# maelaubert/VulkanSift

Hardware: AMD Instinct MI355X
Metric: SIFT detect+match frames/sec (640x480, ~2k kp) (higher is better)
Workload: dtype f32

## Files before the change

include/vksift_hip.h:

```cpp
#ifndef VKSIFT_HIP_H
#define VKSIFT_HIP_H

#include <stddef.h>
#include <stdint.h>

#ifdef __cplusplus
extern "C"
{
#endif

#define VKSIFT_HIP_MAX_TAPS 20
#define VKSIFT_HIP_MATCH_CHUNKS 32
#define VKSIFT_HIP_MATCH_SMALL_NA 1536u
#define VKSIFT_HIP_MATCH_SMALL_NB 4096u
#define VKSIFT_HIP_MATCH_SCRATCH_U32(na, nb) (2u * (size_t)(na) + (size_t)(nb) + 72u + (size_t)(na) * 16u * VKSIFT_HIP_MATCH_CHUNKS)
#define VKSIFT_HIP_ABI_VERSION 6u
#define VKSIFT_HIP_GATHER_SLOTS 512u
#define VKSIFT_HIP_MATCH_SLOTS 256u
#define VKSIFT_HIP_MATCH_PK_NB 32768u
#define VKSIFT_HIP_MAX_ORI 18
#define VKSIFT_HIP_MAX_OCTAVE_SIDE 16383u

  typedef void *vksift_hip_stream;
  typedef void *vksift_hip_graph;
  typedef void *vksift_hip_event;

  int vksift_hip_init(void);
  uint32_t vksift_hip_abi_version(void);
  int vksift_hip_device_count(void);
  int vksift_hip_device_name(int idx, char *out256);
  int vksift_hip_set_device(int idx);
  size_t vksift_hip_device_free_mem(void);
  void *vksift_hip_malloc(size_t bytes);
  void vksift_hip_free(void *p);
  void *vksift_hip_host_malloc(size_t bytes);
  void vksift_hip_host_free(void *p);
  int vksift_hip_host_register(void *p, size_t bytes);
  int vksift_hip_host_unregister(void *p);
  int vksift_hip_is_pinned(const void *p);
  vksift_hip_stream vksift_hip_stream_create(void);
  void vksift_hip_stream_destroy(vksift_hip_stream s);
  int vksift_hip_stream_sync(vksift_hip_stream s);
  int vksift_hip_stream_busy(vksift_hip_stream s);
  vksift_hip_event vksift_hip_event_create(void);
  void vksift_hip_event_destroy(vksift_hip_event e);
  int vksift_hip_event_record(vksift_hip_event e, vksift_hip_stream s);
  int vksift_hip_event_sync(vksift_hip_event e);
  int vksift_hip_event_busy(vksift_hip_event e);
  float vksift_hip_event_elapsed_ms(vksift_hip_event a, vksift_hip_event b);
  int vksift_hip_stream_wait_event(vksift_hip_stream s, vksift_hip_event e);
  int vksift_hip_capture_begin(vksift_hip_stream s);
  int vksift_hip_capture_end(vksift_hip_stream s, vksift_hip_graph *out);
  int vksift_hip_graph_launch(vksift_hip_graph g, vksift_hip_stream s);
  void vksift_hip_graph_destroy(vksift_hip_graph g);
  int vksift_hip_memcpy_h2d(void *dst, const void *src, size_t n, vksift_hip_stream s);
  int vksift_hip_memcpy_d2h(void *dst, const void *src, size_t n, vksift_hip_stream s);
  int vksift_hip_memcpy_d2d(void *dst, const void *src, size_t n, vksift_hip_stream s);
  int vksift_hip_memcpy2d_d2h(void *dst, size_t dpitch, const void *src, size_t spitch, size_t width_bytes, size_t height, vksift_hip_stream s);
  int vksift_hip_post_words(uint32_t *host_mapped_dst, const uint32_t *src, size_t n_words, vksift_hip_stream s);
  int vksift_hip_memset(void *dst, int value, size_t n, vksift_hip_stream s);
  const char *vksift_hip_error_string(int err);
  void vksift_hip_range_push(const char *name);
  void vksift_hip_range_pop(void);

  enum
  {
    VKSIFT_TUNE_WG_TARGET = 0,
    VKSIFT_TUNE_WIDE_MASK = 1,
    VKSIFT_TUNE_MULTI_MAX = 2,
    VKSIFT_TUNE_REFINE_PTR = 3,
    VKSIFT_TUNE_SCAN_FORM = 4,
    VKSIFT_TUNE_PAIR_FORM = 5,
    VKSIFT_TUNE_PYR_GATE = 6,
    VKSIFT_TUNE_DENSE_ROWS = 7,
    VKSIFT_TUNE_SEED_WG = 8,
    VKSIFT_TUNE_SCAN_BAND = 9,
    VKSIFT_TUNE_TAIL_MULTI = 10,
    VKSIFT_TUNE_ZERO_COPY = 11,
    VKSIFT_TUNE_MIN_MARCH = 12,
    VKSIFT_TUNE_COUNT = 16
  };
  int vksift_hip_tune(int knob, int value);
  int vksift_hip_tune_get(int knob);


  typedef struct
  {
    float *base;
    uint32_t w, h;
    uint32_t pitch;
    uint64_t img_stride;
    uint32_t fp16;
    uint32_t reverse;
  } vksift_hip_Plane;

  int vksift_hip_input_blit(const uint8_t *src, uint32_t sw, uint32_t sh, uint64_t src_img_stride, vksift_hip_Plane dst, uint32_t batch,
                            vksift_hip_stream s);

  int vksift_hip_blur(vksift_hip_Plane src, vksift_hip_Plane dst, const float *taps, uint32_t ntaps, uint32_t batch, vksift_hip_stream s);

  int vksift_hip_blur_pair(vksift_hip_Plane src, vksift_hip_Plane dst1, vksift_hip_Plane dst2, const float *taps1, uint32_t ntaps1, const float *taps2,
                           uint32_t ntaps2, uint32_t batch, vksift_hip_stream s);

  int vksift_hip_blur_form(vksift_hip_Plane src, vksift_hip_Plane dst, uint32_t ntaps, uint32_t batch);

  int vksift_hip_blur_multi(const vksift_hip_Plane *src, const vksift_hip_Plane *dst, uint32_t n, const float *taps, uint32_t ntaps, uint32_t batch,
                            vksift_hip_stream s);

  int vksift_hip_blur_downsample(vksift_hip_Plane src, vksift_hip_Plane dst, vksift_hip_Plane next, const float *taps, uint32_t ntaps, uint32_t batch,
                                 vksift_hip_stream s);

  int vksift_hip_seed_upsampled(const uint8_t *src, uint32_t sw, uint32_t sh, uint64_t src_img_stride, vksift_hip_Plane dst, const float *taps, uint32_t ntaps,
                                uint32_t batch, vksift_hip_stream s);

  int vksift_hip_seed_direct(const uint8_t *src, uint32_t sw, uint32_t sh, uint64_t src_img_stride, vksift_hip_Plane dst, const float *taps, uint32_t ntaps,
                             uint32_t batch, vksift_hip_stream s);

  int vksift_hip_downsample(vksift_hip_Plane src, vksift_hip_Plane dst, uint32_t batch, vksift_hip_stream s);

  int vksift_hip_octave_chain(const vksift_hip_Plane *layers, uint32_t n_oct, uint32_t n_layers, uint32_t S, const float *taps, const uint32_t *ntaps,
                              uint32_t batch, vksift_hip_stream s);

  int vksift_hip_dog_plane(const float *lo, const float *hi, uint32_t w, uint32_t h, uint32_t pitch, uint32_t fp16, float *out_dense, vksift_hip_stream s);

  typedef struct
  {
    float *gauss;
    uint32_t fp16;
    uint32_t w, h, pitch;
    uint64_t plane_stride;
    uint64_t img_stride;
    uint32_t S;
    int32_t octave_idx;
    float seed_sigma;
    float dog_threshold;
    float edge_limit;
    uint8_t *feats;
    uint64_t feat_img_stride;
    uint32_t cap;
    uint32_t *found;
    uint32_t found_img_stride;
    uint64_t *seg_mask;
    uint32_t *seg_off;
    uint64_t seg_img_stride;
    uint32_t *cand_xy;
    uint32_t *cand_flag;
    uint32_t *cand_n;
    uint64_t cand_img_stride;
    uint32_t cand_cap;
    float *ori_ang;
    uint32_t *ori_cnt;
    uint64_t ori_img_stride;
    uint32_t max_ori;
    uint32_t use_vlfeat;
    const float *desc_fp_tab;
    uint32_t desc_fp_tab_len;
    uint32_t scan_reverse;
    uint32_t masks_cleared;
    uint32_t sec_index;
  } vksift_hip_OctaveJob;

  typedef struct
  {
    uint8_t *desc;
    uint64_t desc_img_stride;
    uint32_t *norm;
    uint64_t norm_img_stride;
    uint32_t *n;
    uint32_t n_img_stride;
    uint32_t nsec;
    uint32_t sec_cap[16];
    uint8_t *post;
    uint64_t post_img_stride;
    uint32_t *found_post;
    uint32_t found_post_n;
  } vksift_hip_DenseRows;

  int vksift_hip_extract_keypoints(const vksift_hip_OctaveJob *job, uint32_t batch, vksift_hip_stream s, vksift_hip_event scan_done);
  int vksift_hip_orientations(const vksift_hip_OctaveJob *job, uint32_t batch, vksift_hip_stream s);
  int vksift_hip_descriptors(const vksift_hip_OctaveJob *job, uint32_t batch, vksift_hip_stream s);
  int vksift_hip_extract_keypoints_multi(const vksift_hip_OctaveJob *jobs, uint32_t n_jobs, uint32_t batch, vksift_hip_stream s, vksift_hip_event scan_done);
  int vksift_hip_clear_segment_masks(const vksift_hip_OctaveJob *jobs, uint32_t n_jobs, uint32_t batch, vksift_hip_stream s);
  int vksift_hip_selftest_inrange(uint32_t n, uint32_t seed, uint32_t *d_mismatches, vksift_hip_stream s);
  int vksift_hip_orientations_multi(const vksift_hip_OctaveJob *jobs, uint32_t n_jobs, uint32_t batch, vksift_hip_stream s);
  int vksift_hip_descriptors_multi(const vksift_hip_OctaveJob *jobs, uint32_t n_jobs, uint32_t batch, vksift_hip_stream s);
  int vksift_hip_descriptors_multi_dense(const vksift_hip_OctaveJob *jobs, uint32_t n_jobs, uint32_t batch, const vksift_hip_DenseRows *dense,
                                         vksift_hip_stream s);

  int vksift_hip_gather_descriptors(const uint8_t *feats, uint32_t n, uint8_t *desc, vksift_hip_stream s);
  size_t vksift_hip_match_scratch_u32(uint32_t na, uint32_t nb);
  int vksift_hip_match_2nn_desc(const uint8_t *desc_a, uint32_t na, uint32_t a_index_base, const uint8_t *desc_b, uint32_t nb, uint32_t *norm_scratch,
                                size_t scratch_u32, uint8_t *matches, vksift_hip_stream s);
  int vksift_hip_shifted_norms(const uint8_t *desc, uint32_t n, uint32_t *norms, vksift_hip_stream s);
  int vksift_hip_match_2nn_prenormed(const uint8_t *desc_a, const uint32_t *norm_a, uint32_t na, uint32_t a_index_base, const uint8_t *desc_b,
                                     const uint32_t *norm_b, uint32_t nb, uint32_t *scratch, size_t scratch_u32, uint8_t *matches, vksift_hip_stream s);

  int vksift_hip_filter_matches(const uint8_t *fwd, uint64_t fwd_slot_stride, const uint8_t *rev, uint64_t rev_slot_stride, const uint32_t *n_fwd,
                                uint32_t n_stride, float ratio, uint32_t nslots, uint8_t *out, uint64_t out_slot_stride, uint32_t *out_n, vksift_hip_stream s);

  int vksift_hip_pack_features(const uint8_t *feats_base, uint64_t buf_stride, const uint32_t *buf_ids, const uint32_t *out_rows, uint32_t nslots, uint32_t nsec,
                               const uint32_t *sec_off, const uint32_t *sec_cap, const uint32_t *found_base, uint32_t found_buf_stride, uint8_t *out,
                               uint32_t max_rows, uint32_t *found_post, vksift_hip_stream s);
  int vksift_hip_gather_sections(const uint8_t *feats_base, uint64_t buf_stride, const uint32_t *buf_ids, uint32_t nslots, uint32_t nsec,
                                 const uint32_t *sec_off, const uint32_t *sec_cap, const uint32_t *fixed_counts, const uint32_t *found_base,
                                 uint32_t found_buf_stride, uint32_t max_rows, uint32_t pad_rows_to, uint8_t *desc, uint64_t desc_stride,
                                 uint32_t *norms, uint64_t norm_stride, uint32_t *n_out_dev, uint32_t n_stride, vksift_hip_stream s);
  int vksift_hip_match_2nn_async(const uint8_t *cache_desc, const uint32_t *cache_norm, const uint32_t *cache_n, const uint32_t *ids_a, const uint32_t *ids_b,
                                 uint32_t max_na, uint32_t max_nb, uint32_t nb_exact, uint32_t *redo, uint32_t *n_dev, uint8_t *matches, uint32_t nslots, uint64_t cache_desc_stride,
                                 uint64_t cache_norm_stride, uint64_t redo_slot_stride, uint64_t match_slot_stride, uint32_t n_slot_stride,
                                 uint32_t *partial_scratch, vksift_hip_stream s);

  int vksift_hip_gather_correspondences(const uint8_t *feats_base, uint64_t buf_stride, const uint32_t *found_base, uint32_t found_buf_stride,
                                        const uint32_t *slot_tab, const uint32_t *layouts, const uint8_t *filtered, uint64_t filtered_slot_stride,
                                        const uint32_t *filtered_n, uint32_t max_n, uint32_t nslots, float *corr, uint64_t corr_slot_stride, vksift_hip_stream s);
  size_t vksift_hip_ransac_scratch_u32(uint32_t nslots, uint32_t nb_hypotheses);
  int vksift_hip_ransac_homography(const float *corr, uint64_t corr_slot_stride, const uint32_t *n_dev, uint32_t n_stride, uint32_t max_n, uint32_t nslots,
                                   uint32_t nb_hypotheses, float threshold_px, uint64_t seed, uint8_t *results, uint8_t *masks, uint64_t mask_slot_stride,
                                   uint32_t *scratch, size_t scratch_u32, vksift_hip_stream s);
  int vksift_hip_ransac_fundamental(const float *corr, uint64_t corr_slot_stride, const uint32_t *n_dev, uint32_t n_stride, uint32_t max_n, uint32_t nslots,
                                    uint32_t nb_hypotheses, float threshold_px, uint64_t seed, uint8_t *results, uint8_t *masks, uint64_t mask_slot_stride,
                                    uint32_t *scratch, size_t scratch_u32, vksift_hip_stream s);

#define VKSIFT_HIP_GUIDE_HOMOGRAPHY 0u
#define VKSIFT_HIP_GUIDE_FUNDAMENTAL 1u
  int vksift_hip_gather_xy(const uint8_t *feats_base, uint64_t buf_stride, const uint32_t *found_base, uint32_t found_buf_stride, const uint32_t *slot_tab,
                           const uint32_t *layouts, uint32_t max_n, uint32_t nslots, float *xy, uint64_t xy_side_stride, vksift_hip_stream s);
  size_t vksift_hip_guided_scratch_u32(uint32_t nslots, uint32_t max_n);
  int vksift_hip_match_guided(const uint8_t *cache_desc, uint64_t cache_desc_stride, const uint32_t *cache_norm, uint64_t cache_norm_stride, const uint32_t *slot_tab,
                              uint32_t slot_tab_stride, const float *xy, uint64_t xy_side_stride, const uint32_t *n_dev, uint32_t n_stride, uint32_t max_n,
                              const float *models, uint32_t model_stride, const uint32_t *valid, uint32_t valid_stride, uint32_t model_kind, float t2, float ratio,
                              float max_distance, uint32_t cross_check, uint32_t nslots, uint8_t *out, uint64_t out_slot_stride, uint32_t *out_n, uint32_t *scratch,
                              size_t scratch_u32, vksift_hip_stream s);

#ifdef __cplusplus
}
#endif
#endif
```

vulkansift_amd/csrc/hip/extrema.hip:

```cpp
#include <hip/hip_runtime.h>
#include <type_traits>
#include <stdint.h>
#include <stdlib.h>

#include "../detmath.h"
#include "multi.h"
#include "vksift_hip.h"

namespace
{

struct DogView
{
  const float *base;
  int w, h, pitch;
  size_t plane;
  int S;
  int fp16;
};

template <bool F16>
__device__ __forceinline__ float ld(const DogView &d, int s, int x, int y)
{
  if (s < 0 || s > d.S + 1)
// ... 150 lines not shown
    float i33 = ((h11 * h22) - (h12 * h12)) / det;
    oS = -i11 * gS - i12 * gX - i13 * gY;
    oX = -i12 * gS - i22 * gX - i23 * gY;
    oY = -i13 * gS - i23 * gX - i33 * gY;

    if (fabsf(oX) < 0.6f && fabsf(oY) < 0.6f && fabsf(oS) < 0.6f)
      break;
    else if (step < 4)
    {
      rx += ((oX >= 0.6f && rx < (W - 2)) ? 1 : 0) + ((oX <= -0.6f && rx > 1) ? -1 : 0);
      ry += ((oY >= 0.6f && ry < (H - 2)) ? 1 : 0) + ((oY <= -0.6f && ry > 1) ? -1 : 0);
      rs += ((oS >= 0.6f && rs < (S + 1)) ? 1 : 0) + ((oS <= -0.6f && rs > 1) ? -1 : 0);
    }
  }
  float sx = (float)rx + oX, sy = (float)ry + oY, ss = (float)rs + oS;
  float nv = vc + 0.5f * (gX * oX + gY * oY + gS * oS);
  if (!(fabsf(nv) > dog_threshold && fabsf(oX) < 1.5f && fabsf(oY) < 1.5f && fabsf(oS) < 1.5f && sx >= 0 && sx < (float)W && sy >= 0 && sy < (float)H &&
        ss >= 0 && ss <= (float)(S + 1)))
    return false;
  float e11 = xp + xm - 2.f * vc;
  float e22 = yp + ym - 2.f * vc;
  float e12 = h23;
  float edgeness = ((e11 + e22) * (e11 + e22)) / ((e11 * e22) - (e12 * e12));
  if (!((edgeness < edge_limit) && (edgeness >= 0)))
    return false;

  float scale_factor = octave_idx >= 0 ? dm_pow2i(octave_idx) : 1.f / dm_pow2i(-octave_idx);
  kp->scale_x = sx;
  kp->scale_y = sy;
  kp->scale_idx = (uint32_t)roundf(ss);
  kp->octave_idx = octave_idx;
  kp->sigma = seed_sigma * dm_exp2f(ss / (float)S) * scale_factor;
  kp->orientation = 0.f;
  kp->intensity = nv;
  kp->x = sx * scale_factor;
  kp->y = sy * scale_factor;
  return true;
}

struct ExtremaArgs
{
  const float *gauss;
  int fp16;
  int w, h, pitch;
  uint64_t plane_stride, img_stride;
  int S, octave_idx;
  float seed_sigma, dog_threshold, edge_limit;
  uint64_t *seg_mask;
  uint32_t *seg_off;
  uint64_t seg_img_stride;
  int nseg;
  uint8_t *feats;
  uint64_t feat_img_stride;
  uint32_t cap;
  uint32_t *found;
  uint32_t found_img_stride;
  uint32_t *cand_xy;
  uint32_t *cand_flag;
  uint32_t *cand_n;
  uint64_t cand_img_stride;
  uint32_t cand_cap;
  int band;
  uint32_t nsegs;
  uint32_t nchunks;
  int scan_rev;
};

__device__ __forceinline__ float wave_shr1(float v, float edge)
{
  return __builtin_bit_cast(float, __builtin_amdgcn_update_dpp(__builtin_bit_cast(int, edge), __builtin_bit_cast(int, v), 0x138, 0xf, 0xf, false));
}
__device__ __forceinline__ float wave_shl1(float v, float edge)
{
  return __builtin_bit_cast(float, __builtin_amdgcn_update_dpp(__builtin_bit_cast(int, edge), __builtin_bit_cast(int, v), 0x130, 0xf, 0xf, false));
}

__device__ __forceinline__ float fmax2(float a, float b)
{
  float r;
  asm("v_max_f32 %0, %1, %2" : "=v"(r) : "v"(a), "v"(b));
  return r;
}
__device__ __forceinline__ float fmin2(float a, float b)
{
  float r;
  asm("v_min_f32 %0, %1, %2" : "=v"(r) : "v"(a), "v"(b));
  return r;
}
__device__ __forceinline__ float fmax3(float a, float b, float c)
{
  float r;
  asm("v_max3_f32 %0, %1, %2, %3" : "=v"(r) : "v"(a), "v"(b), "v"(c));
  return r;
}
__device__ __forceinline__ float fmin3(float a, float b, float c)
{
  float r;
  asm("v_min3_f32 %0, %1, %2, %3" : "=v"(r) : "v"(a), "v"(b), "v"(c));
  return r;
}

__device__ __forceinline__ unsigned long long spread32(unsigned long long x)
{
  x &= 0xFFFFFFFFull;
  x = (x | (x << 16)) & 0x0000FFFF0000FFFFull;
  x = (x | (x << 8)) & 0x00FF00FF00FF00FFull;
  x = (x | (x << 4)) & 0x0F0F0F0F0F0F0F0Full;
  x = (x | (x << 2)) & 0x3333333333333333ull;
  x = (x | (x << 1)) & 0x5555555555555555ull;
  return x;
}

typedef unsigned u32x2_t __attribute__((ext_vector_type(2)));
constexpr unsigned EXT_OOB = 0x80000000u;

template <int S, int NSLOT, bool F16>
__global__ void __launch_bounds__(256, 4) k_extrema_lean(Multi<ExtremaArgs> m, int strip_major)
{
  const VBlock vb = vblock(m);
  const ExtremaArgs &a = m.oct[vb.o];
  const int band = a.band;
  constexpr int NL = S + 2;
  constexpr int EB = F16 ? 2 : 4;
  constexpr int AHEAD = NSLOT - 3;
  const int lane = threadIdx.x & 63;
  const int wv = __builtin_amdgcn_readfirstlane((int)(threadIdx.x >> 6));
  int b = vb.z;
  int bx = vb.x, by = vb.y * 4 + wv;
  if (strip_major)
  {
    unsigned blk = vb.y * vb.gx + vb.x;
    if (strip_major & 2)
    {
      const unsigned per_img = vb.gx * vb.gy, total = per_img * vb.gz;
      if ((total & 7u) == 0)
      {
        const unsigned n = blk + per_img * vb.z, per = total >> 3, k = n >> 3;
        const unsigned wi = (n & 7u) * per + (a.scan_rev ? per - 1u - k : k);
        b = (int)(wi / per_img);
        blk = wi - (unsigned)b * per_img;
      }
    }
    const unsigned id = blk * 4u + (unsigned)wv, ns = (unsigned)(a.nseg + 1) / 2u;
    by = (int)(id / ns), bx = (int)(id - (unsigned)by * ns);
  }
  const int y0 = by * band;
  if (y0 >= a.h)
    return;
  const int y1 = min(y0 + band, a.h);
  const int x0 = bx * 128, x = x0 + 2 * lane;
  const uint8_t *img = (const uint8_t *)a.gauss + (size_t)b * a.img_stride * EB;
  const int pitch4 = a.pitch * EB;
  __amdgpu_buffer_rsrc_t rs[NL + 1];
#pragma unroll
  for (int l = 0; l <= NL; l++)
    rs[l] = __builtin_amdgcn_make_buffer_rsrc((void *)(img + (size_t)l * a.plane_stride * EB), 0, a.pitch * a.h * EB, 0x00020000);
  const unsigned off2 = x < a.pitch ? (unsigned)x * (unsigned)EB : EXT_OOB;
  const int hx = lane == 0 ? x0 - 1 : x0 + 128;
  const unsigned offh = ((lane == 0 || lane == 63) && hx >= 0 && hx < a.pitch) ? (unsigned)hx * (unsigned)EB : EXT_OOB;
  const unsigned long long colA = __ballot(x >= 1 && x < a.w - 1), colB = __ballot(x + 1 < a.w - 1);
  const float pre = a.dog_threshold * 0.8f;
  const int seg0 = bx * 2;
  const bool has_seg1 = seg0 + 1 < a.nseg;
  const int ylo = max(y0, 1), yhi = min(y1, a.h - 1);
  const bool odd = lane & 1;
  const unsigned half = (unsigned)lane >> 1;

  u32x2_t wv2[NSLOT][NL + 1];
  unsigned wh[NSLOT][NL + 1];
  auto fetch_row = [&](int r, auto SLOT) {
    constexpr int slot = decltype(SLOT)::value;
    const int rr = min(max(r, 0), a.h - 1);
    const int so = rr * pitch4;
#pragma unroll
    for (int l = 0; l <= NL; l++)
    {
      if (F16)
      {
        wv2[slot][l].x = __builtin_amdgcn_raw_buffer_load_b32(rs[l], off2, so, 0);
        wh[slot][l] = (unsigned)__builtin_amdgcn_raw_buffer_load_b16(rs[l], offh, so, 0);
      }
      else
      {
        wv2[slot][l] = __builtin_amdgcn_raw_buffer_load_b64(rs[l], off2, so, 0);
        wh[slot][l] = __builtin_amdgcn_raw_buffer_load_b32(rs[l], offh, so, 0);
      }
    }
  };
  typedef _Float16 h2x __attribute__((ext_vector_type(2)));
  auto to_dog = [&](auto SLOT) {
    constexpr int slot = decltype(SLOT)::value;
    if (F16)
    {
      float lo0, lo1, loh;
      {
        const h2x t = __builtin_bit_cast(h2x, wv2[slot][0].x);
        lo0 = (float)t.x, lo1 = (float)t.y;
        loh = (float)__builtin_bit_cast(h2x, wh[slot][0]).x;
      }
#pragma unroll
      for (int l = 0; l < NL; l++)
      {
        const h2x t = __builtin_bit_cast(h2x, wv2[slot][l + 1].x);
        const float hi0 = (float)t.x, hi1 = (float)t.y, hih = (float)__builtin_bit_cast(h2x, wh[slot][l + 1]).x;
        wv2[slot][l].x = __float_as_uint((float)(_Float16)(hi0 - lo0));
        wv2[slot][l].y = __float_as_uint((float)(_Float16)(hi1 - lo1));
        wh[slot][l] = __float_as_uint((float)(_Float16)(hih - loh));
        lo0 = hi0, lo1 = hi1, loh = hih;
      }
      return;
    }
#pragma unroll
    for (int l = 0; l < NL; l++)
    {
      wv2[slot][l].x = __float_as_uint(__uint_as_float(wv2[slot][l + 1].x) - __uint_as_float(wv2[slot][l].x));
      wv2[slot][l].y = __float_as_uint(__uint_as_float(wv2[slot][l + 1].y) - __uint_as_float(wv2[slot][l].y));
      wh[slot][l] = __float_as_uint(__uint_as_float(wh[slot][l + 1]) - __uint_as_float(wh[slot][l]));
    }
  };

  auto phase = [&](auto PC, int r) {
    constexpr int P = decltype(PC)::value;
    constexpr int sn = P, sm = (P + NSLOT - 1) % NSLOT, so_ = (P + NSLOT - 2) % NSLOT, sf = (P + AHEAD) % NSLOT;
    if (r + AHEAD <= y1)
      fetch_row(r + AHEAD, std::integral_constant<int, sf>{});
    to_dog(std::integral_constant<int, sn>{});
    const int y = r - 1;
    if (y < ylo || y >= yhi)
      return;
    float ownxA[S], ownnA[S], ownxB[S], ownnB[S], fullxA[NL], fullnA[NL], fullxB[NL], fullnB[NL];
#pragma unroll
    for (int l = 0; l < NL; l++)
    {
      const float ao = __uint_as_float(wv2[so_][l].x), am = __uint_as_float(wv2[sm][l].x), an = __uint_as_float(wv2[sn][l].x);
      const float bo = __uint_as_float(wv2[so_][l].y), bm = __uint_as_float(wv2[sm][l].y), bn = __uint_as_float(wv2[sn][l].y);
      const float ho = __uint_as_float(wh[so_][l]), hm = __uint_as_float(wh[sm][l]), hn = __uint_as_float(wh[sn][l]);
      const float vxa = fmax3(ao, am, an), vna = fmin3(ao, am, an);
      const float vxb = fmax3(bo, bm, bn), vnb = fmin3(bo, bm, bn);
      const float vxh = fmax3(ho, hm, hn), vnh = fmin3(ho, hm, hn);
      const float Lx = wave_shr1(vxb, vxh), Ln = wave_shr1(vnb, vnh);
      const float Rx = wave_shl1(vxa, vxh), Rn = wave_shl1(vna, vnh);
      if (l >= 1 && l <= S)
      {
        ownxA[l - 1] = fmax3(Lx, vxb, fmax2(ao, an)), ownnA[l - 1] = fmin3(Ln, vnb, fmin2(ao, an));
        ownxB[l - 1] = fmax3(vxa, Rx, fmax2(bo, bn)), ownnB[l - 1] = fmin3(vna, Rn, fmin2(bo, bn));
      }
      fullxA[l] = fmax3(Lx, vxa, vxb), fullnA[l] = fmin3(Ln, vna, vnb);
      fullxB[l] = fmax3(vxa, vxb, Rx), fullnB[l] = fmin3(vna, vnb, Rn);
    }
#pragma unroll
    for (int sz = 0; sz < S; sz++)
    {
      const int l = sz + 1;
      const float ca = __uint_as_float(wv2[sm][l].x), cb = __uint_as_float(wv2[sm][l].y);
      const float nxa = fmax3(ownxA[sz], fullxA[l - 1], fullxA[l + 1]), nna = fmin3(ownnA[sz], fullnA[l - 1], fullnA[l + 1]);
      const float nxb = fmax3(ownxB[sz], fullxB[l - 1], fullxB[l + 1]), nnb = fmin3(ownnB[sz], fullnB[l - 1], fullnB[l + 1]);
      const unsigned long long ma = (__ballot(ca > nxa) | __ballot(ca < nna)) & __ballot(fabsf(ca) > pre) & colA;
      const unsigned long long mb = (__ballot(cb > nxb) | __ballot(cb < nnb)) & __ballot(fabsf(cb) > pre) & colB;
      if ((ma | mb) != 0ull)
      {
        const unsigned lo = odd ? (unsigned)mb : (unsigned)ma, hi = odd ? (unsigned)(mb >> 32) : (unsigned)(ma >> 32);
        const unsigned long long m0 = __ballot((lo >> half) & 1u), m1 = __ballot((hi >> half) & 1u);
        if (lane == 0)
        {
          const size_t base = ((size_t)sz * a.h + y) * a.nseg + (size_t)b * a.seg_img_stride;
          a.seg_mask[base + seg0] = m0;
          if (has_seg1)
            a.seg_mask[base + seg0 + 1] = m1;
        }
      }
    }
  };

  if (AHEAD >= 1)
    fetch_row(y0 - 1, std::integral_constant<int, 0>{});
  if (AHEAD >= 2)
    fetch_row(y0, std::integral_constant<int, 1 % NSLOT>{});
  int r = y0 - 1;
  for (;;)
  {
    phase(std::integral_constant<int, 0>{}, r);
    if (++r > y1)
      break;
    phase(std::integral_constant<int, 1>{}, r);
    if (++r > y1)
      break;
    phase(std::integral_constant<int, 2>{}, r);
    if (++r > y1)
      break;
    phase(std::integral_constant<int, 3>{}, r);
    if (++r > y1)
      break;
    if (NSLOT > 4)
    {
      phase(std::integral_constant<int, 4 % NSLOT>{}, r);
      if (++r > y1)
        break;
    }
  }
}

constexpr uint32_t SEG_CHUNK = 4096;

__global__ void __launch_bounds__(1024) k_segment_scan(Multi<ExtremaArgs> m)
{
  __shared__ uint32_t wave_tot[16];
  const VBlock vb = vblock(m);
  const ExtremaArgs &a = m.oct[vb.o];
  const int b = (int)vb.y;
  const uint64_t *__restrict__ mask = a.seg_mask + (size_t)b * a.seg_img_stride;
  uint32_t *__restrict__ off = a.seg_off + (size_t)b * a.seg_img_stride;
  uint32_t *__restrict__ chunk_tot = a.cand_flag;
  const uint64_t chunk_img_stride = a.cand_img_stride;
  const uint32_t n = a.nsegs;
  const int lane = threadIdx.x & 63, wave = threadIdx.x >> 6;
  const uint32_t i0 = vb.x * SEG_CHUNK + 4u * threadIdx.x;
  uint32_t p[4];
#pragma unroll
  for (int k = 0; k < 4; k++)
    p[k] = i0 + k < n ? (uint32_t)__popcll(mask[i0 + k]) : 0u;
  const uint32_t tsum = p[0] + p[1] + p[2] + p[3];
  uint32_t incl = tsum;
#pragma unroll
  for (int dlt = 1; dlt < 64; dlt <<= 1)
  {
    uint32_t t = __shfl_up(incl, dlt, 64);
    if (lane >= dlt)
      incl += t;
  }
  if (lane == 63)
    wave_tot[wave] = incl;
  __syncthreads();
  uint32_t wave_base = 0, total = 0;
  for (int wv = 0; wv < 16; wv++)
  {
    if (wv < wave)
      wave_base += wave_tot[wv];
    total += wave_tot[wv];
  }
  uint32_t run = wave_base + incl - tsum;
#pragma unroll
  for (int k = 0; k < 4; k++)
  {
    if (i0 + k < n)
      off[i0 + k] = run;
    run += p[k];
  }
  if (threadIdx.x == 0)
    chunk_tot[(size_t)b * chunk_img_stride + vb.x] = total;
}


__global__ void __launch_bounds__(256) k_cand_list(Multi<ExtremaArgs> mu)
{
  const VBlock vb = vblock(mu);
  const ExtremaArgs &a = mu.oct[vb.o];
  const uint32_t seg = vb.x * 256 + threadIdx.x;
  const int b = (int)vb.y;
  const uint32_t *chunk_tot = a.cand_flag + (size_t)b * a.cand_img_stride;
  if (vb.x == 0 && threadIdx.x == 0)
  {
    uint32_t total = 0;
    for (uint32_t c = 0; c < a.nchunks; c++)
      total += chunk_tot[c];
    a.cand_n[b] = total;
    if (total == 0)
      a.found[(size_t)b * a.found_img_stride] = 0;
  }
  unsigned long long m = seg < a.nsegs ? a.seg_mask[seg + (size_t)b * a.seg_img_stride] : 0ull;
  if (__ballot(m != 0ull) == 0ull)
    return;
  uint32_t base = 0;
  for (uint32_t c = threadIdx.x & 63u, nc = (vb.x * 256u) / SEG_CHUNK; c < nc; c += 64u)
    base += chunk_tot[c];
#pragma unroll
  for (int dlt = 32; dlt >= 1; dlt >>= 1)
    base += __shfl_xor(base, dlt, 64);
  if (m == 0ull)
    return;
  uint32_t pos = a.seg_off[seg + (size_t)b * a.seg_img_stride] + base;
  const uint32_t segx = seg % (uint32_t)a.nseg;
  const uint32_t yy = (seg / (uint32_t)a.nseg) % (uint32_t)a.h;
  const uint32_t sz = seg / ((uint32_t)a.nseg * (uint32_t)a.h);
  uint32_t *out = a.cand_xy + (size_t)b * a.cand_img_stride;
  while (m)
  {
    const int bit = __ffsll((long long)m) - 1;
    m &= m - 1;
    if (pos < a.cand_cap)
      out[pos] = (segx * 64u + (uint32_t)bit) | (yy << 14) | ((sz + 1u) << 28);
    pos++;
  }
}

template <bool F16, bool BUF>
__global__ void __launch_bounds__(256) k_refine_flags(Multi<ExtremaArgs> m)
{
  __shared__ uint32_t s_cnt[4];
  const VBlock vb = vblock(m);
  const ExtremaArgs &a = m.oct[vb.o];
  const int b = (int)vb.x;
  uint32_t n = a.cand_n[b];
  n = n < a.cand_cap ? n : a.cand_cap;
  const uint32_t nch = (n + 255u) / 256u;
  DogView d{(const float *)((const uint8_t *)a.gauss + (size_t)b * a.img_stride * (a.fp16 ? 2u : 4u)), a.w, a.h, a.pitch, (size_t)a.plane_stride, a.S, a.fp16};
  const __amdgpu_buffer_rsrc_t rsrc =
      __builtin_amdgcn_make_buffer_rsrc((void *)d.base, 0, (int)((unsigned)(a.S + 3) * (unsigned)a.plane_stride * (F16 ? 2u : 4u)), 0x00020000);
  const uint32_t *xy = a.cand_xy + (size_t)b * a.cand_img_stride;
  uint32_t *flag = a.cand_flag + (size_t)b * a.cand_img_stride;
  uint32_t *chunk_sum = a.seg_off + (size_t)b * a.seg_img_stride;
  for (uint32_t chunk = vb.y; chunk < nch; chunk += vb.gy)
  {
    const uint32_t i = chunk * 256u + threadIdx.x;
    bool ok = false;
    if (i < n)
    {
      const uint32_t c = xy[i];
      KpRecord kp;
      const int cx = (int)(c & 0x3fffu), cy = (int)((c >> 14) & 0x3fffu), cs = (int)(c >> 28);
      ok = BUF ? refine_texel_buf<F16>(rsrc, a.w, a.h, a.pitch, (unsigned)a.plane_stride, a.S, cx, cy, cs, a.dog_threshold, a.edge_limit, a.seed_sigma, a.octave_idx, &kp)
               : refine_texel<F16>(d, cx, cy, cs, a.dog_threshold, a.edge_limit, a.seed_sigma, a.octave_idx, &kp);
      flag[i] = ok ? 1u : 0u;
    }
    const unsigned long long bal = __ballot(ok);
    if ((threadIdx.x & 63) == 0)
      s_cnt[threadIdx.x >> 6] = (uint32_t)__popcll(bal);
    __syncthreads();
    if (threadIdx.x == 0)
      chunk_sum[chunk] = s_cnt[0] + s_cnt[1] + s_cnt[2] + s_cnt[3];
    __syncthreads();
  }
}

template <bool F16, bool BUF>
__global__ void __launch_bounds__(256) k_cand_emit(Multi<ExtremaArgs> m)
{
  __shared__ uint32_t s_cnt[4];
  __shared__ uint32_t s_red[4];
  __shared__ uint32_t s_list[256];
  const VBlock vb = vblock(m);
  const ExtremaArgs &a = m.oct[vb.o];
  const int b = (int)vb.x;
  const int lane = threadIdx.x & 63, wave = threadIdx.x >> 6;
  uint32_t n = a.cand_n[b];
  n = n < a.cand_cap ? n : a.cand_cap;
  const uint32_t nch = (n + 255u) / 256u;
  DogView d{(const float *)((const uint8_t *)a.gauss + (size_t)b * a.img_stride * (a.fp16 ? 2u : 4u)), a.w, a.h, a.pitch, (size_t)a.plane_stride, a.S, a.fp16};
  const __amdgpu_buffer_rsrc_t rsrc =
      __builtin_amdgcn_make_buffer_rsrc((void *)d.base, 0, (int)((unsigned)(a.S + 3) * (unsigned)a.plane_stride * (F16 ? 2u : 4u)), 0x00020000);
  const uint32_t *xy = a.cand_xy + (size_t)b * a.cand_img_stride;
  const uint32_t *flag = a.cand_flag + (size_t)b * a.cand_img_stride;
  const uint32_t *chunk_sum = a.seg_off + (size_t)b * a.seg_img_stride;
  for (uint32_t chunk = vb.y; chunk < nch; chunk += vb.gy)
  {
    uint32_t part = 0;
    for (uint32_t c = threadIdx.x; c < chunk; c += 256u)
      part += chunk_sum[c];
#pragma unroll
    for (int dlt = 32; dlt >= 1; dlt >>= 1)
      part += __shfl_xor(part, dlt, 64);
    const uint32_t i = chunk * 256u + threadIdx.x;
    const bool v = i < n && flag[i] != 0u;
    const unsigned long long bal = __ballot(v);
    if (lane == 0)
      s_cnt[wave] = (uint32_t)__popcll(bal), s_red[wave] = part;
    __syncthreads();
    const uint32_t cbase = s_red[0] + s_red[1] + s_red[2] + s_red[3];
    uint32_t rank = (uint32_t)__popcll(bal & ((1ull << lane) - 1ull));
    for (int wv = 0; wv < wave; wv++)
      rank += s_cnt[wv];
    const uint32_t total = s_cnt[0] + s_cnt[1] + s_cnt[2] + s_cnt[3];
    if (v)
      s_list[rank] = xy[i];
    __syncthreads();
    const uint32_t idx = cbase + threadIdx.x;
    if (chunk + 1u == nch && threadIdx.x == 0)
      a.found[(size_t)b * a.found_img_stride] = cbase + total;
    if (threadIdx.x < total && idx < a.cap)
    {
      const uint32_t c = s_list[threadIdx.x];
      KpRecord kp;
      const int cx = (int)(c & 0x3fffu), cy = (int)((c >> 14) & 0x3fffu), cs = (int)(c >> 28);
      if (BUF)
        refine_texel_buf<F16>(rsrc, a.w, a.h, a.pitch, (unsigned)a.plane_stride, a.S, cx, cy, cs, a.dog_threshold, a.edge_limit, a.seed_sigma, a.octave_idx, &kp);
      else
        refine_texel<F16>(d, cx, cy, cs, a.dog_threshold, a.edge_limit, a.seed_sigma, a.octave_idx, &kp);
      uint32_t *rec = (uint32_t *)(a.feats + (size_t)b * a.feat_img_stride + (size_t)idx * 164);
      rec[0] = __float_as_uint(kp.x);
      rec[1] = __float_as_uint(kp.y);
      rec[2] = __float_as_uint(kp.scale_x);
      rec[3] = __float_as_uint(kp.scale_y);
      rec[4] = kp.scale_idx;
      rec[5] = (uint32_t)kp.octave_idx;
      rec[6] = __float_as_uint(kp.sigma);
      rec[7] = __float_as_uint(kp.orientation);
      rec[8] = __float_as_uint(kp.intensity);
    }
    __syncthreads();
  }
}

}

static int make_extrema_args(const vksift_hip_OctaveJob *job, ExtremaArgs *out)
{
  if (job->w > VKSIFT_HIP_MAX_OCTAVE_SIDE || job->h > VKSIFT_HIP_MAX_OCTAVE_SIDE || job->S > 14u)
    return (int)hipErrorInvalidValue;
  ExtremaArgs a;
  a.gauss = job->gauss;
  a.fp16 = (int)job->fp16;
  a.w = (int)job->w, a.h = (int)job->h, a.pitch = (int)job->pitch;
  a.plane_stride = job->plane_stride, a.img_stride = job->img_stride;
  a.S = (int)job->S, a.octave_idx = job->octave_idx;
  a.seed_sigma = job->seed_sigma, a.dog_threshold = job->dog_threshold, a.edge_limit = job->edge_limit;
  a.seg_mask = job->seg_mask, a.seg_off = job->seg_off, a.seg_img_stride = job->seg_img_stride;
  a.nseg = (int)((job->w + 63) / 64);
  a.feats = job->feats, a.feat_img_stride = job->feat_img_stride, a.cap = job->cap;
  a.found = job->found, a.found_img_stride = job->found_img_stride;
  a.cand_xy = job->cand_xy, a.cand_flag = job->cand_flag, a.cand_n = job->cand_n;
  a.cand_img_stride = job->cand_img_stride, a.cand_cap = job->cand_cap;
  a.scan_rev = (int)job->scan_reverse;
  a.band = job->h > 256u ? 48 : 16;
  if (vksift_hip_tune_get(VKSIFT_TUNE_SCAN_BAND) > 0 && job->h > 256u)
    a.band = vksift_hip_tune_get(VKSIFT_TUNE_SCAN_BAND);
  a.nsegs = job->S * job->h * (uint32_t)a.nseg;
  a.nchunks = (a.nsegs + SEG_CHUNK - 1u) / SEG_CHUNK;
  if (job->seg_img_stride != a.nsegs || a.nchunks > a.cand_cap)
    return (int)hipErrorInvalidValue;
  *out = a;
  return 0;
}

static int clear_masks(const ExtremaArgs *args, uint32_t n, uint32_t batch, hipStream_t hs)
{
  for (uint32_t i = 0; i < n;)
  {
    uint32_t j = i + 1;
    size_t bytes = sizeof(uint64_t) * (size_t)args[i].nsegs * batch;
    while (j < n && (const uint8_t *)args[j].seg_mask == (const uint8_t *)args[i].seg_mask + bytes)
      bytes += sizeof(uint64_t) * (size_t)args[j].nsegs * batch, j++;
    const hipError_t me = hipMemsetAsync(args[i].seg_mask, 0, bytes, hs);
    if (me != hipSuccess)
      return (int)me;
    i = j;
  }
  return 0;
}

static int extract_run(const vksift_hip_OctaveJob *jobs, uint32_t n, uint32_t batch, hipStream_t hs, hipEvent_t scan_done)
{
  ExtremaArgs args[MULTI_MAX];
  for (uint32_t i = 0; i < n; i++)
  {
    const int e = make_extrema_args(&jobs[i], &args[i]);
    if (e)
      return e;
  }
  const bool f16 = args[0].fp16 != 0;
  const int S = args[0].S;
  {
    uint64_t waves = 0;
    for (uint32_t i = 0; i < n; i++)
      waves += (uint64_t)batch * ((args[i].w + 127) / 128) * ((args[i].h + args[i].band - 1) / args[i].band);
    if (waves < 2048u && vksift_hip_tune_get(VKSIFT_TUNE_SCAN_BAND) <= 0)
      for (uint32_t i = 0; i < n; i++)
        args[i].band = 16;
  }

  bool cleared = true;
  for (uint32_t i = 0; i < n; i++)
    cleared = cleared && jobs[i].masks_cleared != 0;
  if (!cleared)
  {
    const int me = clear_masks(args, n, batch, hs);
    if (me)
      return me;
  }
  const int sm = 3;
  for (uint32_t i = 0; i < n; i++)
    if ((uint64_t)jobs[i].pitch * jobs[i].h * (f16 ? 2u : 4u) >= 0x80000000ull)
      return (int)hipErrorInvalidValue;

#define VKSIFT_MULTI(M, GX, GY, GZ)                              \
  Multi<ExtremaArgs> M;                                           \
  M.n = 0;                                                        \
  for (uint32_t i = 0; i < n; i++)                                \
  {                                                               \
    const ExtremaArgs &a = args[i];                               \
    (void)a;                                                      \
    if (!multi_add(M, args[i], (GX), (GY), (GZ)))                 \
      return (int)hipErrorInvalidValue;                           \
  }
  {
    VKSIFT_MULTI(ms, (uint32_t)(a.nseg + 1) / 2u, ((a.h + a.band - 1) / a.band + 3u) / 4u, batch)
    const dim3 sgrid(ms.start[ms.n]);
    switch (S)
    {
#define VKSIFT_CASE(N)                                                                \
  case N:                                                                             \
    if (f16)                                                                          \
      hipLaunchKernelGGL((k_extrema_lean<N, 5, true>), sgrid, dim3(256), 0, hs, ms, sm);  \
    else                                                                              \
      hipLaunchKernelGGL((k_extrema_lean<N, 4, false>), sgrid, dim3(256), 0, hs, ms, sm); \
    break;
      VKSIFT_CASE(1) VKSIFT_CASE(2) VKSIFT_CASE(3) VKSIFT_CASE(4) VKSIFT_CASE(5) VKSIFT_CASE(6) VKSIFT_CASE(7) VKSIFT_CASE(8) VKSIFT_CASE(9)
      VKSIFT_CASE(10) VKSIFT_CASE(11) VKSIFT_CASE(12) VKSIFT_CASE(13)
#undef VKSIFT_CASE
    default:
      return (int)hipErrorInvalidValue;
    }
  }
  if (scan_done)
    (void)hipEventRecord(scan_done, hs);
  {
    VKSIFT_MULTI(m2, a.nchunks, batch, 1u)
    hipLaunchKernelGGL(k_segment_scan, dim3(m2.start[m2.n]), dim3(1024), 0, hs, m2);
  }
  {
    VKSIFT_MULTI(m3, (a.nsegs + 255u) / 256u, batch, 1u)
    hipLaunchKernelGGL(k_cand_list, dim3(m3.start[m3.n]), dim3(256), 0, hs, m3);
  }
  const uint32_t rcap = 65536u / batch < 16u ? 16u : (65536u / batch > 512u ? 512u : 65536u / batch);
#define VKSIFT_REFINE_CHUNKS(a) (((uint64_t)(a).S * (uint32_t)(a).w * (uint32_t)(a).h / 4u + 64u + 255u) / 256u)
  VKSIFT_MULTI(mr, batch, VKSIFT_REFINE_CHUNKS(a) > rcap ? rcap : (uint32_t)VKSIFT_REFINE_CHUNKS(a), 1u)
#undef VKSIFT_REFINE_CHUNKS
  const dim3 rgrid(mr.start[mr.n]);
  bool buf = vksift_hip_tune_get(VKSIFT_TUNE_REFINE_PTR) == 0;
  for (uint32_t i = 0; i < n; i++)
    buf = buf && (uint64_t)(args[i].S + 3) * args[i].plane_stride * (f16 ? 2u : 4u) < 0x7FFF0000ull;
  if (f16 && buf)
    hipLaunchKernelGGL((k_refine_flags<true, true>), rgrid, dim3(256), 0, hs, mr);
  else if (f16)
    hipLaunchKernelGGL((k_refine_flags<true, false>), rgrid, dim3(256), 0, hs, mr);
  else if (buf)
    hipLaunchKernelGGL((k_refine_flags<false, true>), rgrid, dim3(256), 0, hs, mr);
  else
    hipLaunchKernelGGL((k_refine_flags<false, false>), rgrid, dim3(256), 0, hs, mr);
  if (f16 && buf)
    hipLaunchKernelGGL((k_cand_emit<true, true>), rgrid, dim3(256), 0, hs, mr);
  else if (f16)
    hipLaunchKernelGGL((k_cand_emit<true, false>), rgrid, dim3(256), 0, hs, mr);
  else if (buf)
    hipLaunchKernelGGL((k_cand_emit<false, true>), rgrid, dim3(256), 0, hs, mr);
  else
    hipLaunchKernelGGL((k_cand_emit<false, false>), rgrid, dim3(256), 0, hs, mr);
#undef VKSIFT_MULTI
  return (int)hipGetLastError();
}

extern "C" int vksift_hip_extract_keypoints_multi(const vksift_hip_OctaveJob *jobs, uint32_t n_jobs, uint32_t batch, vksift_hip_stream s,
                                                  vksift_hip_event scan_done)
{
  if (n_jobs == 0 || batch == 0)
    return 0;
  for (uint32_t i0 = 0; i0 < n_jobs;)
  {
    uint32_t i1 = i0 + 1;
    while (i1 < n_jobs && i1 - i0 < multi_run_max() && jobs[i1].S == jobs[i0].S && jobs[i1].fp16 == jobs[i0].fp16)
      i1++;
    const int e = extract_run(jobs + i0, i1 - i0, batch, (hipStream_t)s, i1 == n_jobs ? (hipEvent_t)scan_done : nullptr);
    if (e)
      return e;
    i0 = i1;
  }
  return 0;
}

extern "C" int vksift_hip_clear_segment_masks(const vksift_hip_OctaveJob *jobs, uint32_t n_jobs, uint32_t batch, vksift_hip_stream s)
{
  if (n_jobs == 0 || batch == 0)
    return 0;
  if (n_jobs > 16)
    return (int)hipErrorInvalidValue;
  ExtremaArgs args[16];
  for (uint32_t i = 0; i < n_jobs; i++)
  {
    const int e = make_extrema_args(&jobs[i], &args[i]);
    if (e)
      return e;
  }
  return clear_masks(args, n_jobs, batch, (hipStream_t)s);
}

extern "C" int vksift_hip_extract_keypoints(const vksift_hip_OctaveJob *job, uint32_t batch, vksift_hip_stream s, vksift_hip_event scan_done)
{
  return vksift_hip_extract_keypoints_multi(job, 1, batch, s, scan_done);
}
```

Baseline: 25350.

## Flatten refine/emit grid over actual candidate chunks and restructure segment scan

Splits the segment scan into a chunk-totals kernel and a 1024-thread cand_list kernel that does the in-chunk prefix and skips empty chunks, which removes the seg_off write and read round trip. The refine and emit kernels now build an in-LDS prefix table of real candidate chunks across all octaves and images. Workgroups walk that table by binary search instead of using a fixed per-image grid sized from worst-case estimates, so fewer idle workgroups are launched. The cost is a per-block table build with extra syncs and a large shared-memory footprint, which may reduce occupancy.

Result: no change. 25530, median of 6 (+0.7%).

```diff
diff --git a/include/vksift_hip.h b/include/vksift_hip.h
--- a/include/vksift_hip.h
+++ b/include/vksift_hip.h
@@ -78,6 +78,7 @@
     VKSIFT_TUNE_TAIL_MULTI = 10,
     VKSIFT_TUNE_ZERO_COPY = 11,
     VKSIFT_TUNE_MIN_MARCH = 12,
+    VKSIFT_TUNE_TAIL_GRID = 13,
     VKSIFT_TUNE_COUNT = 16
   };
   int vksift_hip_tune(int knob, int value);
diff --git a/vulkansift_amd/csrc/hip/extrema.hip b/vulkansift_amd/csrc/hip/extrema.hip
--- a/vulkansift_amd/csrc/hip/extrema.hip
+++ b/vulkansift_amd/csrc/hip/extrema.hip
@@ -476,63 +476,54 @@
 
 constexpr uint32_t SEG_CHUNK = 4096;
 
-__global__ void __launch_bounds__(1024) k_segment_scan(Multi<ExtremaArgs> m)
+__device__ __forceinline__ uint32_t chunk_masks(const uint64_t *__restrict__ mask, uint32_t i0, uint32_t n, unsigned long long mk[4], uint32_t p[4])
+{
+#pragma unroll
+  for (int k = 0; k < 4; k++)
+  {
+    mk[k] = i0 + k < n ? mask[i0 + k] : 0ull;
+    p[k] = (uint32_t)__popcll(mk[k]);
+  }
+  return p[0] + p[1] + p[2] + p[3];
+}
+
+__global__ void __launch_bounds__(1024) k_chunk_totals(Multi<ExtremaArgs> m)
 {
   __shared__ uint32_t wave_tot[16];
   const VBlock vb = vblock(m);
   const ExtremaArgs &a = m.oct[vb.o];
   const int b = (int)vb.y;
   const uint64_t *__restrict__ mask = a.seg_mask + (size_t)b * a.seg_img_stride;
-  uint32_t *__restrict__ off = a.seg_off + (size_t)b * a.seg_img_stride;
   uint32_t *__restrict__ chunk_tot = a.cand_flag;
-  const uint64_t chunk_img_stride = a.cand_img_stride;
-  const uint32_t n = a.nsegs;
   const int lane = threadIdx.x & 63, wave = threadIdx.x >> 6;
-  const uint32_t i0 = vb.x * SEG_CHUNK + 4u * threadIdx.x;
+  unsigned long long mk[4];
   uint32_t p[4];
-#pragma unroll
-  for (int k = 0; k < 4; k++)
-    p[k] = i0 + k < n ? (uint32_t)__popcll(mask[i0 + k]) : 0u;
-  const uint32_t tsum = p[0] + p[1] + p[2] + p[3];
-  uint32_t incl = tsum;
-#pragma unroll
-  for (int dlt = 1; dlt < 64; dlt <<= 1)
-  {
-    uint32_t t = __shfl_up(incl, dlt, 64);
-    if (lane >= dlt)
-      incl += t;
-  }
-  if (lane == 63)
-    wave_tot[wave] = incl;
+  uint32_t sum = chunk_masks(mask, vb.x * SEG_CHUNK + 4u * threadIdx.x, a.nsegs, mk, p);
+#pragma unroll
+  for (int dlt = 32; dlt >= 1; dlt >>= 1)
+    sum += __shfl_xor(sum, dlt, 64);
+  if (lane == 0)
+    wave_tot[wave] = sum;
   __syncthreads();
-  uint32_t wave_base = 0, total = 0;
-  for (int wv = 0; wv < 16; wv++)
-  {
-    if (wv < wave)
-      wave_base += wave_tot[wv];
-    total += wave_tot[wv];
-  }
-  uint32_t run = wave_base + incl - tsum;
-#pragma unroll
-  for (int k = 0; k < 4; k++)
-  {
-    if (i0 + k < n)
-      off[i0 + k] = run;
-    run += p[k];
-  }
   if (threadIdx.x == 0)
-    chunk_tot[(size_t)b * chunk_img_stride + vb.x] = total;
-}
-
-
-__global__ void __launch_bounds__(256) k_cand_list(Multi<ExtremaArgs> mu)
-{
+  {
+    uint32_t total = 0;
+    for (int wv = 0; wv < 16; wv++)
+      total += wave_tot[wv];
+    chunk_tot[(size_t)b * a.cand_img_stride + vb.x] = total;
+  }
+}
+
+
+__global__ void __launch_bounds__(1024) k_cand_list(Multi<ExtremaArgs> mu)
+{
+  __shared__ uint32_t wave_tot[16], wave_front[16];
   const VBlock vb = vblock(mu);
   const ExtremaArgs &a = mu.oct[vb.o];
-  const uint32_t seg = vb.x * 256 + threadIdx.x;
   const int b = (int)vb.y;
+  const uint32_t chunk = vb.x;
   const uint32_t *chunk_tot = a.cand_flag + (size_t)b * a.cand_img_stride;
-  if (vb.x == 0 && threadIdx.x == 0)
+  if (chunk == 0 && threadIdx.x == 0)
   {
     uint32_t total = 0;
     for (uint32_t c = 0; c < a.nchunks; c++)
@@ -541,50 +532,163 @@
     if (total == 0)
       a.found[(size_t)b * a.found_img_stride] = 0;
   }
-  unsigned long long m = seg < a.nsegs ? a.seg_mask[seg + (size_t)b * a.seg_img_stride] : 0ull;
-  if (__ballot(m != 0ull) == 0ull)
+  if (chunk_tot[chunk] == 0u)
     return;
-  uint32_t base = 0;
-  for (uint32_t c = threadIdx.x & 63u, nc = (vb.x * 256u) / SEG_CHUNK; c < nc; c += 64u)
-    base += chunk_tot[c];
+  const int lane = threadIdx.x & 63, wave = threadIdx.x >> 6;
+  const uint32_t i0 = chunk * SEG_CHUNK + 4u * threadIdx.x;
+  unsigned long long mk[4];
+  uint32_t p[4];
+  const uint32_t tsum = chunk_masks(a.seg_mask + (size_t)b * a.seg_img_stride, i0, a.nsegs, mk, p);
+  uint32_t incl = tsum;
+#pragma unroll
+  for (int dlt = 1; dlt < 64; dlt <<= 1)
+  {
+    uint32_t t = __shfl_up(incl, dlt, 64);
+    if (lane >= dlt)
+      incl += t;
+  }
+  uint32_t front = 0;
+  for (uint32_t c = threadIdx.x; c < chunk; c += 1024u)
+    front += chunk_tot[c];
 #pragma unroll
   for (int dlt = 32; dlt >= 1; dlt >>= 1)
-    base += __shfl_xor(base, dlt, 64);
-  if (m == 0ull)
+    front += __shfl_xor(front, dlt, 64);
+  if (lane == 63)
+    wave_tot[wave] = incl, wave_front[wave] = front;
+  __syncthreads();
+  if (tsum == 0u)
     return;
-  uint32_t pos = a.seg_off[seg + (size_t)b * a.seg_img_stride] + base;
-  const uint32_t segx = seg % (uint32_t)a.nseg;
-  const uint32_t yy = (seg / (uint32_t)a.nseg) % (uint32_t)a.h;
-  const uint32_t sz = seg / ((uint32_t)a.nseg * (uint32_t)a.h);
+  uint32_t pos = incl - tsum;
+  for (int wv = 0; wv < 16; wv++)
+    pos += wave_front[wv] + (wv < wave ? wave_tot[wv] : 0u);
   uint32_t *out = a.cand_xy + (size_t)b * a.cand_img_stride;
-  while (m)
-  {
-    const int bit = __ffsll((long long)m) - 1;
-    m &= m - 1;
-    if (pos < a.cand_cap)
-      out[pos] = (segx * 64u + (uint32_t)bit) | (yy << 14) | ((sz + 1u) << 28);
-    pos++;
-  }
-}
-
-template <bool F16, bool BUF>
-__global__ void __launch_bounds__(256) k_refine_flags(Multi<ExtremaArgs> m)
-{
-  __shared__ uint32_t s_cnt[4];
+#pragma unroll
+  for (int k = 0; k < 4; k++)
+  {
+    unsigned long long m = mk[k];
+    if (m == 0ull)
+      continue;
+    const uint32_t seg = i0 + (uint32_t)k;
+    const uint32_t segx = seg % (uint32_t)a.nseg;
+    const uint32_t yy = (seg / (uint32_t)a.nseg) % (uint32_t)a.h;
+    const uint32_t sz = seg / ((uint32_t)a.nseg * (uint32_t)a.h);
+    while (m)
+    {
+      const int bit = __ffsll((long long)m) - 1;
+      m &= m - 1;
+      if (pos < a.cand_cap)
+        out[pos] = (segx * 64u + (uint32_t)bit) | (yy << 14) | ((sz + 1u) << 28);
+      pos++;
+    }
+  }
+}
+
+constexpr uint32_t CHUNK_TAB_MAX = 4096;
+
+struct ChunkWalk
+{
+  uint32_t tab[CHUNK_TAB_MAX + 1];
+  uint32_t wave_tot[4];
+};
+
+__device__ uint32_t chunk_table(const Multi<ExtremaArgs> &m, uint32_t batch, ChunkWalk &w)
+{
+  const uint32_t N = (uint32_t)m.n * batch;
+  for (int o = 0; o < m.n; o++)
+  {
+    const ExtremaArgs &a = m.oct[o];
+    for (uint32_t b = threadIdx.x; b < batch; b += 256u)
+    {
+      uint32_t n = a.cand_n[b];
+      n = n < a.cand_cap ? n : a.cand_cap;
+      w.tab[(uint32_t)o * batch + b] = (n + 255u) / 256u;
+    }
+  }
+  __syncthreads();
+  const uint32_t per = (N + 255u) / 256u, e0 = threadIdx.x * per, e1 = e0 + per < N ? e0 + per : N;
+  const int lane = threadIdx.x & 63, wave = threadIdx.x >> 6;
+  uint32_t tsum = 0;
+  for (uint32_t e = e0; e < e1; e++)
+    tsum += w.tab[e];
+  uint32_t incl = tsum;
+#pragma unroll
+  for (int dlt = 1; dlt < 64; dlt <<= 1)
+  {
+    uint32_t t = __shfl_up(incl, dlt, 64);
+    if (lane >= dlt)
+      incl += t;
+  }
+  if (lane == 63)
+    w.wave_tot[wave] = incl;
+  __syncthreads();
+  uint32_t run = incl - tsum;
+  for (int wv = 0; wv < wave; wv++)
+    run += w.wave_tot[wv];
+  for (uint32_t e = e0; e < e1; e++)
+  {
+    const uint32_t c = w.tab[e];
+    w.tab[e] = run;
+    run += c;
+  }
+  const uint32_t total = w.wave_tot[0] + w.wave_tot[1] + w.wave_tot[2] + w.wave_tot[3];
+  if (threadIdx.x == 0)
+    w.tab[N] = total;
+  __syncthreads();
+  return total;
+}
+
+__device__ __forceinline__ uint32_t chunk_pair(const ChunkWalk &w, uint32_t N, uint32_t f)
+{
+  uint32_t lo = 0, hi = N;
+  while (hi - lo > 1u)
+  {
+    const uint32_t mid = (lo + hi) >> 1;
+    if (w.tab[mid] <= f)
+      lo = mid;
+    else
+      hi = mid;
+  }
+  return lo;
+}
+
+template <typename Body>
+__device__ __forceinline__ void walk_chunks(const Multi<ExtremaArgs> &m, uint32_t batch, ChunkWalk &w, Body body)
+{
+  if (batch != 0u)
+  {
+    const uint32_t total = chunk_table(m, batch, w), N = (uint32_t)m.n * batch;
+    for (uint32_t f = blockIdx.x; f < total; f += gridDim.x)
+    {
+      const uint32_t e = (uint32_t)__builtin_amdgcn_readfirstlane((int)chunk_pair(w, N, f));
+      const uint32_t o = e / batch;
+      body(m.oct[o], (int)(e - o * batch), f - w.tab[e]);
+    }
+    return;
+  }
   const VBlock vb = vblock(m);
   const ExtremaArgs &a = m.oct[vb.o];
   const int b = (int)vb.x;
   uint32_t n = a.cand_n[b];
   n = n < a.cand_cap ? n : a.cand_cap;
   const uint32_t nch = (n + 255u) / 256u;
-  DogView d{(const float *)((const uint8_t *)a.gauss + (size_t)b * a.img_stride * (a.fp16 ? 2u : 4u)), a.w, a.h, a.pitch, (size_t)a.plane_stride, a.S, a.fp16};
-  const __amdgpu_buffer_rsrc_t rsrc =
-      __builtin_amdgcn_make_buffer_rsrc((void *)d.base, 0, (int)((unsigned)(a.S + 3) * (unsigned)a.plane_stride * (F16 ? 2u : 4u)), 0x00020000);
-  const uint32_t *xy = a.cand_xy + (size_t)b * a.cand_img_stride;
-  uint32_t *flag = a.cand_flag + (size_t)b * a.cand_img_stride;
-  uint32_t *chunk_sum = a.seg_off + (size_t)b * a.seg_img_stride;
   for (uint32_t chunk = vb.y; chunk < nch; chunk += vb.gy)
-  {
+    body(a, b, chunk);
+}
+
+template <bool F16, bool BUF>
+__global__ void __launch_bounds__(256) k_refine_flags(Multi<ExtremaArgs> m, uint32_t batch)
+{
+  __shared__ ChunkWalk s_walk;
+  __shared__ uint32_t s_cnt[4];
+  walk_chunks(m, batch, s_walk, [&](const ExtremaArgs &a, int b, uint32_t chunk) {
+    uint32_t n = a.cand_n[b];
+    n = n < a.cand_cap ? n : a.cand_cap;
+    DogView d{(const float *)((const uint8_t *)a.gauss + (size_t)b * a.img_stride * (a.fp16 ? 2u : 4u)), a.w, a.h, a.pitch, (size_t)a.plane_stride, a.S, a.fp16};
+    const __amdgpu_buffer_rsrc_t rsrc =
+        __builtin_amdgcn_make_buffer_rsrc((void *)d.base, 0, (int)((unsigned)(a.S + 3) * (unsigned)a.plane_stride * (F16 ? 2u : 4u)), 0x00020000);
+    const uint32_t *xy = a.cand_xy + (size_t)b * a.cand_img_stride;
+    uint32_t *flag = a.cand_flag + (size_t)b * a.cand_img_stride;
+    uint32_t *chunk_sum = a.seg_off + (size_t)b * a.seg_img_stride;
     const uint32_t i = chunk * 256u + threadIdx.x;
     bool ok = false;
     if (i < n)
@@ -603,30 +707,27 @@
     if (threadIdx.x == 0)
       chunk_sum[chunk] = s_cnt[0] + s_cnt[1] + s_cnt[2] + s_cnt[3];
     __syncthreads();
-  }
+  });
 }
 
 template <bool F16, bool BUF>
-__global__ void __launch_bounds__(256) k_cand_emit(Multi<ExtremaArgs> m)
-{
+__global__ void __launch_bounds__(256) k_cand_emit(Multi<ExtremaArgs> m, uint32_t batch)
+{
+  __shared__ ChunkWalk s_walk;
   __shared__ uint32_t s_cnt[4];
   __shared__ uint32_t s_red[4];
   __shared__ uint32_t s_list[256];
-  const VBlock vb = vblock(m);
-  const ExtremaArgs &a = m.oct[vb.o];
-  const int b = (int)vb.x;
   const int lane = threadIdx.x & 63, wave = threadIdx.x >> 6;
-  uint32_t n = a.cand_n[b];
-  n = n < a.cand_cap ? n : a.cand_cap;
-  const uint32_t nch = (n + 255u) / 256u;
-  DogView d{(const float *)((const uint8_t *)a.gauss + (size_t)b * a.img_stride * (a.fp16 ? 2u : 4u)), a.w, a.h, a.pitch, (size_t)a.plane_stride, a.S, a.fp16};
-  const __amdgpu_buffer_rsrc_t rsrc =
-      __builtin_amdgcn_make_buffer_rsrc((void *)d.base, 0, (int)((unsigned)(a.S + 3) * (unsigned)a.plane_stride * (F16 ? 2u : 4u)), 0x00020000);
-  const uint32_t *xy = a.cand_xy + (size_t)b * a.cand_img_stride;
-  const uint32_t *flag = a.cand_flag + (size_t)b * a.cand_img_stride;
-  const uint32_t *chunk_sum = a.seg_off + (size_t)b * a.seg_img_stride;
-  for (uint32_t chunk = vb.y; chunk < nch; chunk += vb.gy)
-  {
+  walk_chunks(m, batch, s_walk, [&](const ExtremaArgs &a, int b, uint32_t chunk) {
+    uint32_t n = a.cand_n[b];
+    n = n < a.cand_cap ? n : a.cand_cap;
+    const uint32_t nch = (n + 255u) / 256u;
+    DogView d{(const float *)((const uint8_t *)a.gauss + (size_t)b * a.img_stride * (a.fp16 ? 2u : 4u)), a.w, a.h, a.pitch, (size_t)a.plane_stride, a.S, a.fp16};
+    const __amdgpu_buffer_rsrc_t rsrc =
+        __builtin_amdgcn_make_buffer_rsrc((void *)d.base, 0, (int)((unsigned)(a.S + 3) * (unsigned)a.plane_stride * (F16 ? 2u : 4u)), 0x00020000);
+    const uint32_t *xy = a.cand_xy + (size_t)b * a.cand_img_stride;
+    const uint32_t *flag = a.cand_flag + (size_t)b * a.cand_img_stride;
+    const uint32_t *chunk_sum = a.seg_off + (size_t)b * a.seg_img_stride;
     uint32_t part = 0;
     for (uint32_t c = threadIdx.x; c < chunk; c += 256u)
       part += chunk_sum[c];
@@ -671,7 +772,7 @@
       rec[8] = __float_as_uint(kp.intensity);
     }
     __syncthreads();
-  }
+  });
 }
 
 }
@@ -788,36 +889,46 @@
     (void)hipEventRecord(scan_done, hs);
   {
     VKSIFT_MULTI(m2, a.nchunks, batch, 1u)
-    hipLaunchKernelGGL(k_segment_scan, dim3(m2.start[m2.n]), dim3(1024), 0, hs, m2);
-  }
-  {
-    VKSIFT_MULTI(m3, (a.nsegs + 255u) / 256u, batch, 1u)
-    hipLaunchKernelGGL(k_cand_list, dim3(m3.start[m3.n]), dim3(256), 0, hs, m3);
-  }
+    hipLaunchKernelGGL(k_chunk_totals, dim3(m2.start[m2.n]), dim3(1024), 0, hs, m2);
+    hipLaunchKernelGGL(k_cand_list, dim3(m2.start[m2.n]), dim3(1024), 0, hs, m2);
+  }
+  const int tail_grid = vksift_hip_tune_get(VKSIFT_TUNE_TAIL_GRID);
+  const bool flat = tail_grid >= 0 && (uint64_t)n * batch <= CHUNK_TAB_MAX;
   const uint32_t rcap = 65536u / batch < 16u ? 16u : (65536u / batch > 512u ? 512u : 65536u / batch);
 #define VKSIFT_REFINE_CHUNKS(a) (((uint64_t)(a).S * (uint32_t)(a).w * (uint32_t)(a).h / 4u + 64u + 255u) / 256u)
   VKSIFT_MULTI(mr, batch, VKSIFT_REFINE_CHUNKS(a) > rcap ? rcap : (uint32_t)VKSIFT_REFINE_CHUNKS(a), 1u)
 #undef VKSIFT_REFINE_CHUNKS
-  const dim3 rgrid(mr.start[mr.n]);
+  uint32_t wgs = mr.start[mr.n];
+  if (flat)
+  {
+    uint64_t most = 0;
+    for (uint32_t i = 0; i < n; i++)
+      most += (uint64_t)batch * ((args[i].cand_cap + 255u) / 256u);
+    wgs = (uint64_t)n * batch * 128u < 8192u ? n * batch * 128u : 8192u;
+    wgs = tail_grid > 0 ? (uint32_t)tail_grid : wgs;
+    wgs = most < wgs ? (uint32_t)most : wgs;
+  }
+  const dim3 rgrid(wgs);
+  const uint32_t wbatch = flat ? batch : 0u;
   bool buf = vksift_hip_tune_get(VKSIFT_TUNE_REFINE_PTR) == 0;
   for (uint32_t i = 0; i < n; i++)
     buf = buf && (uint64_t)(args[i].S + 3) * args[i].plane_stride * (f16 ? 2u : 4u) < 0x7FFF0000ull;
   if (f16 && buf)
-    hipLaunchKernelGGL((k_refine_flags<true, true>), rgrid, dim3(256), 0, hs, mr);
+    hipLaunchKernelGGL((k_refine_flags<true, true>), rgrid, dim3(256), 0, hs, mr, wbatch);
   else if (f16)
-    hipLaunchKernelGGL((k_refine_flags<true, false>), rgrid, dim3(256), 0, hs, mr);
+    hipLaunchKernelGGL((k_refine_flags<true, false>), rgrid, dim3(256), 0, hs, mr, wbatch);
   else if (buf)
-    hipLaunchKernelGGL((k_refine_flags<false, true>), rgrid, dim3(256), 0, hs, mr);
+    hipLaunchKernelGGL((k_refine_flags<false, true>), rgrid, dim3(256), 0, hs, mr, wbatch);
   else
-    hipLaunchKernelGGL((k_refine_flags<false, false>), rgrid, dim3(256), 0, hs, mr);
+    hipLaunchKernelGGL((k_refine_flags<false, false>), rgrid, dim3(256), 0, hs, mr, wbatch);
   if (f16 && buf)
-    hipLaunchKernelGGL((k_cand_emit<true, true>), rgrid, dim3(256), 0, hs, mr);
+    hipLaunchKernelGGL((k_cand_emit<true, true>), rgrid, dim3(256), 0, hs, mr, wbatch);
   else if (f16)
-    hipLaunchKernelGGL((k_cand_emit<true, false>), rgrid, dim3(256), 0, hs, mr);
+    hipLaunchKernelGGL((k_cand_emit<true, false>), rgrid, dim3(256), 0, hs, mr, wbatch);
   else if (buf)
-    hipLaunchKernelGGL((k_cand_emit<false, true>), rgrid, dim3(256), 0, hs, mr);
+    hipLaunchKernelGGL((k_cand_emit<false, true>), rgrid, dim3(256), 0, hs, mr, wbatch);
   else
-    hipLaunchKernelGGL((k_cand_emit<false, false>), rgrid, dim3(256), 0, hs, mr);
+    hipLaunchKernelGGL((k_cand_emit<false, false>), rgrid, dim3(256), 0, hs, mr, wbatch);
 #undef VKSIFT_MULTI
   return (int)hipGetLastError();
 }
```
